# cruiseresearchgroup/ViLCo

Measured on AMD Instinct MI355X. Metric: clips/sec (fwd+bwd) MQ transformer T=2304 C=2304, higher is better.
Workload: dtype fp16 MFMA on 2-part splits of power-of-two scaled fp32 operands (22 significant bits, 3 MFMAs per product), fp32 accumulate: fp32-equivalent; weight-gradient products with contraction length >= 2048 use the leading fp16 parts only (11-bit operands, 1 MFMA; <= 3.5e-4 of the 3-MFMA gradients at this c; 1 GPU; MQ ViLCo backbone config P: T=2304 Cin=2304 D=1024 H=16 arch(2,2,5) XLNet layer text L=77x768 22 classes, train mode with the reference's dropout 0.1 / droppath 0.1 / XLNet dropout 0.1 (mq_vilco.yaml, xlnet_config_1024.json); clips_per_gpu=2, global_batch=2, parallelism=dp1

## Files before the change

### include/vilco_hip.h

```cpp
#ifndef VILCO_HIP_H
#define VILCO_HIP_H

#include <stddef.h>
#include <stdint.h>

#ifdef __cplusplus
extern "C" {
#endif

enum vilco_status {
  VILCO_OK = 0,
  VILCO_ERR_BADARG = -1,
  VILCO_ERR_UNSUPPORTED = -2,
  VILCO_ERR_LAUNCH = -3,
  VILCO_ERR_WORKSPACE = -4
};

const char* vilco_status_str(int status);
const char* vilco_version(void);
size_t vilco_abi_sizeof(const char* struct_name);

enum { VILCO_ACT_NONE = 0, VILCO_ACT_RELU = 1, VILCO_ACT_GELU = 2 };
enum { VILCO_TAP_NONE = 0, VILCO_TAP_A = 1, VILCO_TAP_B = 2 };

// ... 252 lines not shown
                    float* partial, float* norm_coef, void* stream);
typedef struct vilco_optim_desc {
  int32_t kind;
  const int64_t* ptrs;
  const int64_t* numel;
  const int32_t* chunk_tensor;
  const int64_t* chunk_off;
  const int32_t* group;
  int32_t n, nchunks, chunk;
  const float* lr;
  const float* wd;
  int32_t ngroups;
  float beta1, beta2, eps, momentum;
  const float* tensor_step;
  const float* norm_coef;
  float* chunk_amax;
  const float* lr_dev;
} vilco_optim_desc;
int vilco_optim_step(const vilco_optim_desc* d, void* stream);
int vilco_store_f32(float* dst, const float* vals, int32_t n, void* stream);

int vilco_qkv_pre_supported(int32_t C);
int vilco_qkv_pre_amax_parts(int32_t B, int32_t T, int32_t stride);
int vilco_qkv_pre_fwd(const float* x, const float* ln1_g, const float* ln1_b, const float* const* w,
                      const float* const* gam, const float* const* bet, const int32_t* len, float* h,
                      float* const* y, float* mean1, float* rstd1, float* const* mean, float* const* rstd,
                      float* const* amax_parts, int32_t B, int32_t T, int32_t C, int32_t stride, float eps1, float eps,
                      void* stream);
size_t vilco_qkv_pre_bwd_workspace(int32_t B, int32_t T, int32_t C, int32_t stride);
int vilco_qkv_pre_bwd(const float* h, const float* const* w, const float* const* gam, const float* const* dy,
                      const float* const* mean, const float* const* rstd, const int32_t* len,
                      const float* dh_ext, float* const* dc, float* dh, float* dparams, int32_t B, int32_t T,
                      int32_t C, int32_t stride, void* workspace, size_t workspace_bytes, void* stream);

typedef struct vilco_loss_desc {
  const float* logits;
  const float* offsets;
  const float* level_scale;
  const float* points;
  const int32_t* row_level;
  const int32_t* row_pos;
  const int32_t* level_len;
  const float* gt;
  const float* gauss;
  float* loss_norm;
  int32_t B, R, C, L, Nmax;
  float center_radius, label_smoothing, momentum, loss_weight, al_weight;
  int32_t use_al;
} vilco_loss_desc;
size_t vilco_mq_loss_workspace(int32_t B, int32_t R, int32_t C);
int vilco_mq_loss_fwd(const vilco_loss_desc* d, float* out, float* saved, void* almax_state, void* workspace,
                      size_t workspace_bytes, void* stream);
int vilco_mq_loss_bwd(const vilco_loss_desc* d, const float* g_cls, const float* g_reg, const float* g_al,
                      const float* g_final, const float* saved, const void* workspace, float* d_logits,
                      float* d_offsets, float* d_level_scale, float* d_gauss, void* stream);

typedef struct vilco_distill_desc {
  const float* logits;
  const float* targets;
  const int32_t* level_row;
  const int32_t* level_T;
  const int32_t* level_dev;
  int32_t B, R, C, L;
  int32_t clip;
  int32_t ldt;
  int32_t n_known;
// ... 138 lines not shown
```

### vilco_amd/_lib.py

```python
import ctypes as C
import os

_HERE = os.path.dirname(os.path.abspath(__file__))
LIB_PATH = os.environ.get("VILCO_HIP_LIB") or os.path.join(_HERE, "libvilco_hip.so")

ACT_NONE, ACT_RELU, ACT_GELU = 0, 1, 2
TAP_NONE, TAP_A, TAP_B = 0, 1, 2

c_fp = C.c_void_p
i32, i64, f32, sz = C.c_int32, C.c_int64, C.c_float, C.c_size_t


class GemmDesc(C.Structure):
    _cname_ = "vilco_gemm_desc"
    _fields_ = [
        ("A", c_fp), ("B", c_fp), ("C", c_fp),
        ("M", i32), ("N", i32), ("K", i32),
        ("a_kcontig", i32), ("b_kcontig", i32),
        ("lda", i64), ("ldb", i64), ("ldc", i64),
        ("batch_outer", i32), ("batch_inner", i32),
        ("sAo", i64), ("sAi", i64), ("sBo", i64), ("sBi", i64), ("sCo", i64), ("sCi", i64),
        ("tap_operand", i32), ("tapC", i32), ("tapT", i32),
        ("precision", i32),
        ("alpha", f32), ("beta", f32),
# ... 70 lines not shown
                ("rows", i64), ("C", i32), ("drop_p", f32), ("drop_seed", C.c_uint32),
                ("workspace", c_fp), ("workspace_bytes", sz), ("amax_parts", c_fp), ("n_parts", c_fp),
                ("dy_amax", c_fp), ("n_dy_amax", i32), ("planes", c_fp), ("planes_bytes", sz), ("seq_len", i32),
                ("row_mask", c_fp)]


class OptimDesc(C.Structure):
    _cname_ = "vilco_optim_desc"
    _fields_ = [("kind", i32), ("ptrs", c_fp), ("numel", c_fp), ("chunk_tensor", c_fp), ("chunk_off", c_fp), ("group", c_fp),
                ("n", i32), ("nchunks", i32), ("chunk", i32), ("lr", c_fp), ("wd", c_fp), ("ngroups", i32),
                ("beta1", f32), ("beta2", f32), ("eps", f32), ("momentum", f32), ("tensor_step", c_fp), ("norm_coef", c_fp),
                ("chunk_amax", c_fp), ("lr_dev", c_fp)]


class DistillDesc(C.Structure):
    _cname_ = "vilco_distill_desc"
    _fields_ = [("logits", c_fp), ("targets", c_fp), ("level_row", c_fp), ("level_T", c_fp), ("level_dev", c_fp),
                ("B", i32), ("R", i32), ("C", i32), ("L", i32), ("clip", i32), ("ldt", i32), ("n_known", i32), ("mode", i32),
                ("scale", f32)]


class BicCorrectDesc(C.Structure):
    _cname_ = "vilco_bic_correct_desc"
    _fields_ = [("x", c_fp), ("y", c_fp), ("splits", c_fp), ("table", c_fp), ("rows", i64), ("C", i32), ("S", i32),
                ("ldx", i32), ("ldy", i32), ("n_layers", i32)]


class PromptDesc(C.Structure):
    _cname_ = "vilco_prompt_desc"
    _fields_ = [("x", c_fp), ("prompt", c_fp), ("key", c_fp), ("cls", c_fp), ("idx_in", c_fp),
                ("B", i32), ("L", i32), ("C", i32), ("P", i32), ("len", i32), ("k", i32), ("key_mode", i32), ("vote", i32),
                ("idx", c_fp), ("sim", c_fp), ("pn", c_fp), ("xn", c_fp), ("selkey", c_fp), ("prompted", c_fp),
                ("reduce_sim", c_fp), ("workspace", c_fp), ("workspace_bytes", sz)]


SIGNATURES = {
    "vilco_status_str": (C.c_char_p, [C.c_int]),
    "vilco_version": (C.c_char_p, []),
    "vilco_abi_sizeof": (sz, [C.c_char_p]),
    "vilco_defer_set": (C.c_int, [i32]),
    "vilco_defer_pending": (i64, []),
    "vilco_defer_flush": (C.c_int, [c_fp]),
    "vilco_gemm_workspace": (sz, [C.POINTER(GemmDesc)]),
    "vilco_gemm": (C.c_int, [C.POINTER(GemmDesc), c_fp]),
    "vilco_gemm_group": (C.c_int, [C.POINTER(GemmDesc), i32, c_fp]),
    "vilco_gemm_amax_parts": (i32, [C.POINTER(GemmDesc)]),
    "vilco_gemm_force": (C.c_int, [i32, i32]),
    "vilco_gemm_set_skinny": (C.c_int, [i32]),
    "vilco_gemm_config_gen": (i64, []),
    "vilco_gemm_profile_begin": (C.c_int, []),
    "vilco_gemm_profile_end": (C.c_int, [C.POINTER(C.c_double), C.POINTER(C.c_int64)]),
    "vilco_gemm_profile_records": (C.c_int64, [C.POINTER(C.c_int64), C.POINTER(C.c_double), C.c_int64]),
    "vilco_pack_bytes": (sz, [i64, i64, i32]),
    "vilco_pack_item_bytes": (sz, [C.POINTER(PackItem), i32]),
    "vilco_pack": (C.c_int, [c_fp, i64, i64, i64, i32, c_fp, sz, c_fp]),
    "vilco_pack_many": (C.c_int, [C.POINTER(PackItem), i32, i32, c_fp]),
    "vilco_layernorm_fwd": (C.c_int, [C.POINTER(LnFwdDesc), c_fp]),
    "vilco_layernorm_planes_bytes": (sz, [i64, i32, i32]),
    "vilco_layernorm_bwd_workspace": (sz, [i64, i32]),
    "vilco_layernorm_bwd": (C.c_int, [C.POINTER(LnBwdDesc), c_fp]),
    "vilco_dwconv3_fwd": (C.c_int, [c_fp, c_fp, c_fp, c_fp, i32, i32, i32, i32, c_fp]),
    "vilco_dwconv3_bwd_workspace": (sz, [i32, i32, i32, i32]),
    "vilco_dwconv3_bwd": (C.c_int, [c_fp, c_fp, c_fp, c_fp, c_fp, c_fp, i32, i32, i32, i32, c_fp, sz, c_fp]),
    "vilco_maxpool3s2_fwd": (C.c_int, [c_fp, c_fp, c_fp, i32, i32, i32, c_fp]),
    "vilco_maxpool3s2_bwd": (C.c_int, [c_fp, c_fp, c_fp, c_fp, i32, i32, i32, c_fp]),
    "vilco_softmax_fwd": (C.c_int, [c_fp, c_fp, i32, i32, i32, i32, i32, c_fp]),
# ... 10 lines not shown
    "vilco_attn_dsplanes_bytes": (sz, [i32, i32, i32]),
    "vilco_xl_scores_workspace": (sz, [i32, i32, i32, i32]),
    "vilco_xl_scores": (C.c_int, [c_fp, c_fp, c_fp, i32, i32, i32, i32, i32, i32, c_fp, sz, c_fp]),
    "vilco_decode_workspace": (sz, [i32, i32]),
    "vilco_decode": (C.c_int, [c_fp, c_fp, c_fp, c_fp, c_fp, i32, i32, i32, f32, f32, c_fp, c_fp, c_fp, c_fp, c_fp, sz, c_fp]),
    "vilco_scale_add_fwd": (C.c_int, [c_fp, c_fp, c_fp, c_fp, c_fp, c_fp, i32, i32, i32, i32, c_fp]),
    "vilco_colsum_workspace": (sz, [i64, i32]),
    "vilco_scale_add_bwd": (C.c_int, [C.POINTER(ScaleAddBwdDesc), c_fp]),
    "vilco_dropout": (C.c_int, [c_fp, c_fp, i64, f32, C.c_uint32, C.c_uint64, c_fp]),
    "vilco_attn_dropout_mask": (C.c_int, [c_fp, i64, i32, f32, C.c_uint32, c_fp]),
    "vilco_seed_word_set": (C.c_int, [C.c_uint32, c_fp]),
    "vilco_seed_word_bump": (C.c_int, [c_fp]),
    "vilco_seed_word_get": (C.c_int, [C.POINTER(C.c_uint32)]),
    "vilco_axpby": (C.c_int, [c_fp, c_fp, c_fp, f32, f32, i64, c_fp]),
    "vilco_act_bwd": (C.c_int, [C.POINTER(ActBwdDesc), c_fp]),
    "vilco_act_bwd_planes_bytes": (sz, [i64, i32, i32]),
    "vilco_colsum": (C.c_int, [c_fp, c_fp, i64, i32, c_fp, sz, c_fp]),
    "vilco_mask_rows": (C.c_int, [c_fp, c_fp, i32, i32, i32, c_fp]),
    "vilco_add_pe": (C.c_int, [c_fp, c_fp, c_fp, c_fp, i32, i32, i32, c_fp]),
    "vilco_transpose2d": (C.c_int, [c_fp, c_fp, i32, i32, i32, c_fp]),
    "vilco_permute3": (C.c_int, [c_fp, c_fp, i32, i32, i32, i64, i64, i64, i64, c_fp]),
    "vilco_grad_norm": (C.c_int, [c_fp, c_fp, c_fp, c_fp, i32, i32, i32, f32, c_fp, c_fp, c_fp]),
    "vilco_optim_step": (C.c_int, [C.POINTER(OptimDesc), c_fp]),
    "vilco_store_f32": (C.c_int, [c_fp, C.POINTER(f32), i32, c_fp]),
    "vilco_qkv_pre_supported": (C.c_int, [i32]),
    "vilco_qkv_pre_amax_parts": (C.c_int, [i32, i32, i32]),
    "vilco_qkv_pre_fwd": (C.c_int, [c_fp, c_fp, c_fp, C.POINTER(c_fp), C.POINTER(c_fp), C.POINTER(c_fp), c_fp, c_fp,
                                    C.POINTER(c_fp), c_fp, c_fp, C.POINTER(c_fp), C.POINTER(c_fp), C.POINTER(c_fp), i32, i32,
                                    i32, i32, f32, f32, c_fp]),
    "vilco_qkv_pre_bwd_workspace": (sz, [i32, i32, i32, i32]),
    "vilco_qkv_pre_bwd": (C.c_int, [c_fp, C.POINTER(c_fp), C.POINTER(c_fp), C.POINTER(c_fp), C.POINTER(c_fp),
                                    C.POINTER(c_fp), c_fp, c_fp, C.POINTER(c_fp), c_fp, c_fp, i32, i32, i32, i32, c_fp, sz,
                                    c_fp]),
    "vilco_mq_loss_workspace": (sz, [i32, i32, i32]),
    "vilco_mq_loss_fwd": (C.c_int, [C.POINTER(LossDesc), c_fp, c_fp, c_fp, c_fp, sz, c_fp]),
    "vilco_mq_loss_bwd": (C.c_int, [C.POINTER(LossDesc), c_fp, c_fp, c_fp, c_fp, c_fp, c_fp, c_fp, c_fp, c_fp, c_fp,
                                    c_fp]),
    "vilco_cl_distill_workspace": (sz, [i64]),
    "vilco_cl_distill_fwd": (C.c_int, [C.POINTER(DistillDesc), c_fp, c_fp, sz, c_fp]),
    "vilco_cl_distill_bwd": (C.c_int, [C.POINTER(DistillDesc), c_fp, c_fp, c_fp]),
    "vilco_cl_penalty": (C.c_int, [c_fp, c_fp, c_fp, c_fp, i32, i32, i32, f32, i32, c_fp, c_fp, c_fp]),
    "vilco_cl_accumulate": (C.c_int, [c_fp, c_fp, c_fp, c_fp, i32, i32, i32, i32, f32, f32, c_fp]),
    "vilco_nms_workspace": (sz, [i64, i32]),
    "vilco_nms_1d": (C.c_int, [c_fp, c_fp, c_fp, i32, i64, f32, c_fp, c_fp, c_fp, sz, c_fp]),
    "vilco_softnms_1d": (C.c_int, [c_fp, c_fp, c_fp, i32, i64, f32, f32, f32, i32, i64, c_fp, c_fp, c_fp,
                                   c_fp, sz, c_fp]),
    "vilco_nms_set_kernel": (C.c_int, [i32]),
    "vilco_nms_last_kernels": (C.c_int, []),
    "vilco_det_ap_workspace": (sz, [i64, i32, i32]),
    "vilco_det_ap": (C.c_int, [c_fp, c_fp, c_fp, c_fp, c_fp, i64, c_fp, c_fp, c_fp, c_fp, c_fp, i32, i32, c_fp, i32, i32,
                               C.POINTER(C.c_double), i32, c_fp, c_fp, c_fp, sz, c_fp]),
    "vilco_retrieval_hits_workspace": (sz, [i32, i32, i32]),
    "vilco_retrieval_hits": (C.c_int, [c_fp, c_fp, c_fp, c_fp, c_fp, c_fp, c_fp, i32, C.POINTER(C.c_double), i32,
                                       C.POINTER(i32), i32, c_fp, c_fp, c_fp, sz, c_fp]),
    "vilco_score_fuse_workspace": (sz, [i64, i32]),
    "vilco_score_fuse": (C.c_int, [c_fp, c_fp, c_fp, C.POINTER(i32), i64, i32, c_fp, i32, i32, i32, C.POINTER(i32), i64,
                                   c_fp, c_fp, c_fp, c_fp, c_fp, c_fp, sz, c_fp]),
    "vilco_nlq_recall_workspace": (sz, [i64, i32]),
    "vilco_nlq_recall": (C.c_int, [c_fp, i32, c_fp, i32, c_fp, c_fp, i64, i32, C.POINTER(C.c_double), i32, C.POINTER(i32), i32,
                                   i32, c_fp, c_fp, c_fp, c_fp, c_fp, c_fp, sz, c_fp]),
    "vilco_nlq_ensemble": (C.c_int, [c_fp, i32, c_fp, i32, i64, i32, i32, i32, C.c_double, C.c_double, i32, i32, c_fp, c_fp,
                                     c_fp, c_fp, c_fp]),
    "vilco_frob_scale_workspace": (sz, [i64, i64]),
    "vilco_frob_scale": (C.c_int, [c_fp, i64, i64, i64, c_fp, c_fp, sz, c_fp]),
    "vilco_gram_workspace": (sz, [i64, i64]),
    "vilco_gram": (C.c_int, [c_fp, i64, i64, i64, c_fp, c_fp, i32, c_fp, sz, c_fp]),
# ... 51 lines not shown
```

### vilco_amd/csrc/qkvpre.hip

```cpp
#include <cstdlib>
#include "common.h"

void vilco_reduce_rows(const float* ws, float* out0, float* out1, int nrows, int ncols, int split, hipStream_t s);

namespace {

constexpr int QT = 256;

struct QkvArgs {
  const float* x;
  const float* g1; const float* b1;
  const float* w[3];
  const float* gam[3]; const float* bet[3];
  const int* len;
  float* h;
  float* y[3];
  float* mean1; float* rstd1;
  float* mean[3]; float* rstd[3];
  float* amax[3];
  int B, T, Tout, C, stride, seg;
  float eps1, eps;
};

template <int N, int NW>
// ... 609 lines not shown
#pragma unroll
  for (int i = 0; i < 6; ++i) p[(long)i * C + c] = acc[i];
#pragma unroll
  for (int j = 0; j < 3; ++j)
#pragma unroll
    for (int k = 0; k < 3; ++k) p[(long)(6 + 3 * j) * C + c * 3 + k] = acc[6 + 3 * j + k];
}

__global__ __launch_bounds__(QT) void qkv_pre_bwd_dh_kernel(QkvBwdArgs a, const float* __restrict__ dh_ext, float* __restrict__ dh) {
  const int C = a.C, C4 = C >> 2, s = a.stride;
  const long total = (long)a.B * a.T * C4;
  for (long i = (long)blockIdx.x * blockDim.x + threadIdx.x; i < total; i += (long)gridDim.x * blockDim.x) {
    const int c = (int)(i % C4) * 4;
    const long bt = i / C4;
    const int t = (int)(bt % a.T), b = (int)(bt / a.T);
    float4 o = dh_ext ? *reinterpret_cast<const float4*>(dh_ext + bt * C + c) : make_float4(0.f, 0.f, 0.f, 0.f);
#pragma unroll
    for (int tap = 0; tap < 3; ++tap) {
      const int num = t + 1 - tap;
      if (num < 0 || (num % s) != 0) continue;
      const int to = num / s;
      if (to >= a.Tout) continue;
      const long r = (long)b * a.Tout + to;
#pragma unroll
      for (int j = 0; j < 3; ++j) {
        const float4 g = *reinterpret_cast<const float4*>(a.dc[j] + r * C + c);
        const float* wj = a.w[j] + c * 3 + tap;
        o.x += wj[0] * g.x; o.y += wj[3] * g.y; o.z += wj[6] * g.z; o.w += wj[9] * g.w;
      }
    }
    *reinterpret_cast<float4*>(dh + bt * C + c) = o;
  }
}

int pick_seg(int B, int Tout) {
  int seg = 32;
  while (seg > 4 && (long)B * ((Tout + seg - 1) / seg) < 512) seg >>= 1;
  return seg;
}

bool bad_common(int B, int T, int C, int stride) {
  return B < 0 || T < 0 || C <= 0 || (stride != 1 && stride != 2) || (T % stride) != 0;
}

int param_blocks(long rows) {
  long b = (rows + 31) / 32;
  if (b > 96) b = 96;
  return b < 1 ? 1 : (int)b;
}

}

extern "C" int vilco_qkv_pre_supported(int32_t C) { return C > 0 && (C % 256) == 0 && C / 256 <= 9; }

#define QKV_CASE(KERNEL, CPT_, NT_, GRID, ...) hipLaunchKernelGGL((KERNEL<CPT_, NT_>), GRID, dim3(NT_), 0, s, __VA_ARGS__)
#define QKV_DISPATCH(C_, KERNEL, GRID, ...)                                                                          \
  do {                                                                                                              \
    const int cpt256 = (C_) / 256;                                                                                  \
    if (cpt256 > 4 && (C_) % 768 == 0 && (C_) / 768 <= 4) {                                                         \
      switch ((C_) / 768) {                                                                                         \
        case 1: QKV_CASE(KERNEL, 1, 768, GRID, __VA_ARGS__); break;                                                 \
        case 2: QKV_CASE(KERNEL, 2, 768, GRID, __VA_ARGS__); break;                                                 \
        case 3: QKV_CASE(KERNEL, 3, 768, GRID, __VA_ARGS__); break;                                                 \
        default: QKV_CASE(KERNEL, 4, 768, GRID, __VA_ARGS__); break;                                                \
      }                                                                                                             \
    } else {                                                                                                        \
// ... 106 lines not shown
  return (size_t)param_blocks((long)B * (T / stride)) * 15 * (size_t)C * sizeof(float);
}

extern "C" int vilco_qkv_pre_bwd(const float* h, const float* const* w, const float* const* gam, const float* const* dy,
                                 const float* const* mean, const float* const* rstd, const int32_t* len,
                                 const float* dh_ext, float* const* dc, float* dh, float* dparams, int32_t B, int32_t T,
                                 int32_t C, int32_t stride, void* workspace, size_t workspace_bytes, void* stream) {
  if (!h || !w || !gam || !dy || !mean || !rstd || !len || !dc || !dh || !dparams || bad_common(B, T, C, stride))
    return VILCO_ERR_BADARG;
  if (!vilco_qkv_pre_supported(C)) return VILCO_ERR_UNSUPPORTED;
  if (B == 0 || T == 0) return VILCO_OK;
  if (!workspace || workspace_bytes < vilco_qkv_pre_bwd_workspace(B, T, C, stride)) return VILCO_ERR_WORKSPACE;
  hipStream_t s = reinterpret_cast<hipStream_t>(stream);
  QkvBwdArgs a;
  a.h = h; a.len = len;
  for (int j = 0; j < 3; ++j) {
    if (!w[j] || !dy[j] || !mean[j] || !rstd[j] || !dc[j]) return VILCO_ERR_BADARG;
    a.w[j] = w[j]; a.gam[j] = gam[j]; a.dy[j] = dy[j]; a.mean[j] = mean[j]; a.rstd[j] = rstd[j]; a.dc[j] = dc[j];
  }
  a.B = B; a.T = T; a.Tout = T / stride; a.C = C; a.stride = stride; a.seg = pick_seg(B, a.Tout);
  const dim3 grid((a.Tout + a.seg - 1) / a.seg, B);
  QKV_DISPATCH(C, qkv_pre_bwd_rows_kernel, grid, a);
  const long rows = (long)B * a.Tout;
  const int nb = param_blocks(rows);
  const int rpb = (int)((rows + nb - 1) / nb);
  float* partial = reinterpret_cast<float*>(workspace);
  hipLaunchKernelGGL(qkv_pre_bwd_params_kernel, dim3(nb, (C + QT - 1) / QT), dim3(QT), 0, s, a, partial, rpb);
  vilco_reduce_rows(partial, dparams, nullptr, nb, 15 * C, 15 * C, s);
  long blocks = ((long)B * T * (C / 4) + QT - 1) / QT;
  if (blocks > 4096) blocks = 4096;
  hipLaunchKernelGGL(qkv_pre_bwd_dh_kernel, dim3((int)blocks), dim3(QT), 0, s, a, dh_ext, dh);
  return vilco_launch_status();
}
```

### vilco_amd/csrc/status.hip

```cpp
#include <string.h>
#include "common.h"

extern "C" const char* vilco_status_str(int status) {
  switch (status) {
    case VILCO_OK: return "ok";
    case VILCO_ERR_BADARG: return "vilco_hip: bad argument (null pointer, negative size or misaligned operand)";
    case VILCO_ERR_UNSUPPORTED: return "vilco_hip: shape not supported by the gfx950 kernels";
    case VILCO_ERR_LAUNCH: return "vilco_hip: kernel launch failed";
    case VILCO_ERR_WORKSPACE: return "vilco_hip: workspace too small";
    default: return "vilco_hip: unknown status";
  }
}

extern "C" const char* vilco_version(void) { return "vilco_hip 0.1 gfx950"; }

extern "C" size_t vilco_abi_sizeof(const char* struct_name) {
#define ABI_SIZE(T) if (struct_name && !strcmp(struct_name, #T)) return sizeof(T);
  ABI_SIZE(vilco_gemm_desc) ABI_SIZE(vilco_pack_item) ABI_SIZE(vilco_attn_amax_in) ABI_SIZE(vilco_loss_desc)
  ABI_SIZE(vilco_ln_fwd_desc) ABI_SIZE(vilco_ln_bwd_desc) ABI_SIZE(vilco_attn_desc) ABI_SIZE(vilco_scale_add_bwd_desc)
  ABI_SIZE(vilco_act_bwd_desc) ABI_SIZE(vilco_optim_desc) ABI_SIZE(vilco_distill_desc) ABI_SIZE(vilco_bic_correct_desc)
  ABI_SIZE(vilco_prompt_desc)
#undef ABI_SIZE
  return 0;
}

__device__ int32_t vilco_status_word_storage[16];

int32_t* vilco_status_word_dev() {
  static int32_t* p = [] {
    void* q = nullptr;
    if (hipGetSymbolAddress(&q, HIP_SYMBOL(vilco_status_word_storage)) != hipSuccess) q = nullptr;
    return reinterpret_cast<int32_t*>(q);
  }();
  return p;
}

extern "C" int vilco_status_word_take(int32_t* out) {
  if (!out) return VILCO_ERR_BADARG;
  if (hipDeviceSynchronize() != hipSuccess) return VILCO_ERR_LAUNCH;
  if (hipMemcpyFromSymbol(out, HIP_SYMBOL(vilco_status_word_storage), sizeof(int32_t)) != hipSuccess) return VILCO_ERR_LAUNCH;
  const int32_t zero = 0;
  return hipMemcpyToSymbol(HIP_SYMBOL(vilco_status_word_storage), &zero, sizeof(int32_t)) == hipSuccess ? VILCO_OK : VILCO_ERR_LAUNCH;
}
```

### vilco_amd/ops.py

```python
import ctypes as C
import math
import os

import torch

from . import _lib
from ._lib import ACT_GELU, ACT_NONE, ACT_RELU, TAP_A, TAP_B, TAP_NONE, GemmDesc

_PRECISIONS = {"split": 0, 0: 0, "bf16": 1, 1: 1, "split3": 2, "fp32": 2, 2: 2, "f16x2": 3, 3: 3}
DEFAULT_PRECISION = _PRECISIONS[os.environ.get("VILCO_PRECISION", "f16x2")]
_precision = DEFAULT_PRECISION


_DW = {"f16x1": 4, "f16x2": None}
dw_precision = _DW[os.environ.get("VILCO_DW_PRECISION", "f16x1")]
DW_FAST_MIN_K = 2048


def _dw_prec(prec, K=0):
    return dw_precision if (dw_precision is not None and prec == 3 and K >= DW_FAST_MIN_K) else prec


def set_precision(p=None):
    global _precision
    _precision = DEFAULT_PRECISION if p is None else _PRECISIONS[p]


def arithmetic_key():
    return (int(_precision), -1 if dw_precision is None else int(dw_precision), int(DW_FAST_MIN_K), bool(producer_planes),
            bool(ln_planes), bool(attn_planes), bool(produce_amax), bool(conv_tap_planes), bool(defer_finish), bool(use_qkv_pre),
            tuple(sorted(_FORKS)), int(_dw_fork_rows),
            bool(fold_skip_grads), bool(xl_ds_planes), bool(xl_scores_kernel), bool(linear_group_enabled), bool(use_flash),
            bool(_reuse_packs), bool(_weight_cache), str(range_check), int(_lib.load().vilco_gemm_config_gen()), bool(pack_group_enabled), bool(conv_dz_planes), bool(ln_bwd_amax),
            bool(fused_prompt))


def get_precision():
    return _precision


_raw_stream = getattr(torch._C, "_cuda_getCurrentRawStream", None)


def _stream():
    if _raw_stream is not None:
        return _raw_stream(torch.cuda.current_device())
    return torch.cuda.current_stream().cuda_stream


def _p(t):
    return None if t is None else t.data_ptr()


grad_slot_provider = None


def _grad_out(w):
    if grad_slot_provider is not None:
        slot = grad_slot_provider(w)
        if slot is not None and slot.shape == w.shape and slot.is_contiguous():
            return slot
    return torch.empty_like(w)

# ... 2018 lines not shown
    _chk(ab)
    lib = _lib.load()
    out = torch.empty(3, dtype=torch.float64, device=logits.device)
    nws = lib.vilco_bic_eval_ws_bytes(N, n_clips, int(lo), int(hi))
    ws = _ws(nws, logits.device)
    _lib.check(lib.vilco_bic_eval(logits.data_ptr(), label_bits.data_ptr(), weight.data_ptr(), pos.data_ptr(), clip_ptr.data_ptr(),
                                  N, n_clips, Cn, int(lo), int(hi), float(smoothing), ab.data_ptr(), out.data_ptr(), ws.data_ptr(),
                                  nws, _stream()))
    return out


def bic_fit(logits, label_bits, weight, pos, clip_ptr, order, batch_clips, lo, hi, smoothing, lr, ab):
    N, Cn, n_clips = _bic_cache_args(logits, label_bits, weight, pos, clip_ptr)
    _chk(ab)
    if not order.is_cuda or order.dtype != torch.int32 or not order.is_contiguous():
        raise RuntimeError("order must be a contiguous int32 tensor on the device")
    lib = _lib.load()
    batch_clips = int(batch_clips)
    n_steps = int(order.numel()) // batch_clips if batch_clips > 0 else 0
    losses = torch.empty(n_steps, dtype=torch.float64, device=logits.device)
    nws = lib.vilco_bic_fit_ws_bytes(N, n_clips, batch_clips, int(lo), int(hi))
    ws = _ws(nws, logits.device)
    _lib.check(lib.vilco_bic_fit(logits.data_ptr(), label_bits.data_ptr(), weight.data_ptr(), pos.data_ptr(), clip_ptr.data_ptr(),
                                 N, n_clips, order.data_ptr(), n_steps, batch_clips, Cn, int(lo), int(hi), float(smoothing),
                                 float(lr), ab.data_ptr(), losses.data_ptr(), ws.data_ptr(), nws, _stream()))
    return losses


def qkv_pre_supported(Cn):
    return bool(_lib.load().vilco_qkv_pre_supported(int(Cn)))


use_qkv_pre = os.environ.get("VILCO_QKV_PRE", "1") != "0"


def _ptr3(ts):
    return (_lib.c_fp * 3)(*[_p(t) for t in ts])


class _QkvPre(torch.autograd.Function):

    @staticmethod
    def forward(ctx, x, g1, b1, wq, wk, wv, gq, bq, gk, bk, gv, bv, lens, stride, eps1, eps, want_h, skip=False):
        _chk(x, g1, b1, wq, wk, wv, gq, bq, gk, bk, gv, bv)
        ctx.skip = bool(skip)
        ctx.set_materialize_grads(False)
        lib = _lib.load()
        B, T, Cn = x.shape
        To = T // stride
        dev = x.device
        ys = [torch.empty(B, To, Cn, dtype=torch.float32, device=dev) for _ in range(3)]
        h = torch.empty_like(x) if want_h else None
        stats1 = torch.empty(2, B * T, dtype=torch.float32, device=dev)
        stats = torch.empty(6, B * To, dtype=torch.float32, device=dev)
        means, rstds = [stats[2 * j] for j in range(3)], [stats[2 * j + 1] for j in range(3)]
        npart = lib.vilco_qkv_pre_amax_parts(B, T, int(stride)) if (produce_amax and _precision == 3) else 0
        parts = torch.empty(3, npart, dtype=torch.float32, device=dev) if npart > 0 else None
        _lib.check(lib.vilco_qkv_pre_fwd(x.data_ptr(), _p(g1), _p(b1), _ptr3([wq, wk, wv]), _ptr3([gq, gk, gv]),
                                         _ptr3([bq, bk, bv]), lens.data_ptr(), _p(h), _ptr3(ys), stats1[0].data_ptr(),
                                         stats1[1].data_ptr(), _ptr3(means), _ptr3(rstds),
                                         _ptr3([parts[0], parts[1], parts[2]]) if parts is not None else None, B, T, Cn,
                                         int(stride), float(eps1), float(eps), _stream()))
        if parts is not None:
            for j in range(3):
                _leave(_QkvPre, j, amax=(parts[j], npart))
        ctx.stride, ctx.eps1, ctx.want_h = int(stride), float(eps1), bool(want_h)
        ctx.save_for_backward(x, g1, b1, wq, wk, wv, gq, gk, gv, lens, stats1, stats, h)
        outs = (ys[0], ys[1], ys[2], h) if want_h else (ys[0], ys[1], ys[2])
        return outs + (x,) if skip else outs

    @staticmethod
    def backward(ctx, dq, dk, dv, *more):
        x, g1, b1, wq, wk, wv, gq, gk, gv, lens, stats1, stats, h = ctx.saved_tensors
        more = list(more)
        dh_ext = more.pop(0) if ctx.want_h and more else None
        dskip = more.pop(0) if ctx.skip and more else None
        dskip = None if dskip is None else dskip.contiguous()
        lib = _lib.load()
        B, T, Cn = x.shape
        To = T // ctx.stride
        dev = x.device
        if h is None:
            h = torch.empty_like(x)
            d = _lib.LnFwdDesc(x=x.data_ptr(), gamma=_p(g1), beta=_p(b1), y=h.data_ptr(), rows=B * T, C=Cn, eps=ctx.eps1)
            _lib.check(lib.vilco_layernorm_fwd(C.byref(d), _stream()))
        dys = [torch.zeros(B, To, Cn, dtype=torch.float32, device=dev) if g is None else g.contiguous() for g in (dq, dk, dv)]
        dcs = [torch.empty(B, To, Cn, dtype=torch.float32, device=dev) for _ in range(3)]
        dh = torch.empty_like(x)
        dpar = torch.empty(15, Cn, dtype=torch.float32, device=dev)
        nws = lib.vilco_qkv_pre_bwd_workspace(B, T, Cn, ctx.stride)
        means, rstds = [stats[2 * j] for j in range(3)], [stats[2 * j + 1] for j in range(3)]
        dh_ext = None if dh_ext is None else dh_ext.contiguous()
        dx = torch.empty_like(x)
        dg1 = torch.empty(Cn, dtype=torch.float32, device=dev)
        db1 = torch.empty(Cn, dtype=torch.float32, device=dev)
        with _Deferring(g1, wq, wk, wv, gq, gk, gv) as dfr:
            ws = _ws(nws, dev)
            _lib.check(lib.vilco_qkv_pre_bwd(h.data_ptr(), _ptr3([wq, wk, wv]), _ptr3([gq, gk, gv]), _ptr3(dys), _ptr3(means),
                                             _ptr3(rstds), lens.data_ptr(), _p(dh_ext), _ptr3(dcs), dh.data_ptr(), dpar.data_ptr(),
                                             B, T, Cn, ctx.stride, ws.data_ptr(), nws, _stream()))
            del dcs
            ws1 = _ws(lib.vilco_layernorm_bwd_workspace(B * T, Cn), dev)
            d = _lib.LnBwdDesc(dy=dh.data_ptr(), x=x.data_ptr(), gamma=_p(g1), mean=stats1[0].data_ptr(), rstd=stats1[1].data_ptr(),
                               dres=_p(dskip), dx=dx.data_ptr(), dgamma=dg1.data_ptr(), dbeta=db1.data_ptr(), rows=B * T, C=Cn,
                               workspace=ws1.data_ptr(), workspace_bytes=ws1.numel())
            _lib.check(lib.vilco_layernorm_bwd(C.byref(d), _stream()))
            dfr.hold(dpar, dg1, db1)
        dws = [dpar[6 + 3 * j:9 + 3 * j].view_as(w) for j, w in enumerate((wq, wk, wv))]
        dgs = [dpar[2 * j].view_as(g) for j, g in enumerate((gq, gk, gv))]
        dbs = [dpar[2 * j + 1].view_as(g) for j, g in enumerate((gq, gk, gv))]
        return (dx, dg1.view_as(g1), db1.view_as(g1), dws[0], dws[1], dws[2], dgs[0], dbs[0], dgs[1], dbs[1], dgs[2], dbs[2],
                None, None, None, None, None, None)


# ... 119 lines not shown
```

Baseline: 99.96 clips/s.

## Fuse QKV pre-norm backward with LN1 backward into one streaming kernel

Adds a fused backward kernel for the LN1 -> depthwise conv (q/k/v) -> LN path at stride 2. It recomputes the normalized input on the fly from x and the saved stats, streams over time with a sliding window, and computes the conv/LN gradients, the LN1 input gradient (including skip and external dh), and per-block parameter partials in one pass. This removes the materialized h recompute, the dc/dh intermediates, and the separate LN backward launch, cutting HBM traffic and launch count. In exchange it adds register pressure and serial per-row block reductions, and applies only to stride 2.

Result: no change. 100.8 clips/s (median of 3 runs) (+0.8%).

```diff
diff --git a/include/vilco_hip.h b/include/vilco_hip.h
--- a/include/vilco_hip.h
+++ b/include/vilco_hip.h
@@ -308,6 +308,32 @@
                       const float* const* mean, const float* const* rstd, const int32_t* len,
                       const float* dh_ext, float* const* dc, float* dh, float* dparams, int32_t B, int32_t T,
                       int32_t C, int32_t stride, void* workspace, size_t workspace_bytes, void* stream);
+
+typedef struct vilco_qkv_pre_bwd_desc {
+  const float* x;
+  const float* gamma1;
+  const float* beta1;
+  const float* mean1;
+  const float* rstd1;
+  const float* w[3];
+  const float* gam[3];
+  const float* dy[3];
+  const float* mean[3];
+  const float* rstd[3];
+  const int32_t* len;
+  const float* dh_ext;
+  const float* dskip;
+  float* dx;
+  float* dparams;
+  float* dgamma1;
+  float* dbeta1;
+  int32_t B, T, C, stride;
+  void* workspace;
+  size_t workspace_bytes;
+} vilco_qkv_pre_bwd_desc;
+int vilco_qkv_pre_bwd_fused_supported(int32_t C, int32_t stride);
+size_t vilco_qkv_pre_bwd_fused_workspace(int32_t B, int32_t T, int32_t C, int32_t stride);
+int vilco_qkv_pre_bwd_fused(const vilco_qkv_pre_bwd_desc* d, void* stream);
 
 typedef struct vilco_loss_desc {
   const float* logits;
diff --git a/vilco_amd/_lib.py b/vilco_amd/_lib.py
--- a/vilco_amd/_lib.py
+++ b/vilco_amd/_lib.py
@@ -126,6 +126,15 @@
                 ("B", i32), ("L", i32), ("C", i32), ("P", i32), ("len", i32), ("k", i32), ("key_mode", i32), ("vote", i32),
                 ("idx", c_fp), ("sim", c_fp), ("pn", c_fp), ("xn", c_fp), ("selkey", c_fp), ("prompted", c_fp),
                 ("reduce_sim", c_fp), ("workspace", c_fp), ("workspace_bytes", sz)]
+
+
+class QkvPreBwdDesc(C.Structure):
+    _cname_ = "vilco_qkv_pre_bwd_desc"
+    _fields_ = [("x", c_fp), ("gamma1", c_fp), ("beta1", c_fp), ("mean1", c_fp), ("rstd1", c_fp),
+                ("w", c_fp * 3), ("gam", c_fp * 3), ("dy", c_fp * 3), ("mean", c_fp * 3), ("rstd", c_fp * 3),
+                ("len", c_fp), ("dh_ext", c_fp), ("dskip", c_fp), ("dx", c_fp), ("dparams", c_fp), ("dgamma1", c_fp),
+                ("dbeta1", c_fp), ("B", i32), ("T", i32), ("C", i32), ("stride", i32),
+                ("workspace", c_fp), ("workspace_bytes", sz)]
 
 
 SIGNATURES = {
@@ -202,6 +211,9 @@
     "vilco_qkv_pre_bwd": (C.c_int, [c_fp, C.POINTER(c_fp), C.POINTER(c_fp), C.POINTER(c_fp), C.POINTER(c_fp),
                                     C.POINTER(c_fp), c_fp, c_fp, C.POINTER(c_fp), c_fp, c_fp, i32, i32, i32, i32, c_fp, sz,
                                     c_fp]),
+    "vilco_qkv_pre_bwd_fused_supported": (C.c_int, [i32, i32]),
+    "vilco_qkv_pre_bwd_fused_workspace": (sz, [i32, i32, i32, i32]),
+    "vilco_qkv_pre_bwd_fused": (C.c_int, [C.POINTER(QkvPreBwdDesc), c_fp]),
     "vilco_mq_loss_workspace": (sz, [i32, i32, i32]),
     "vilco_mq_loss_fwd": (C.c_int, [C.POINTER(LossDesc), c_fp, c_fp, c_fp, c_fp, sz, c_fp]),
     "vilco_mq_loss_bwd": (C.c_int, [C.POINTER(LossDesc), c_fp, c_fp, c_fp, c_fp, c_fp, c_fp, c_fp, c_fp, c_fp, c_fp,
diff --git a/vilco_amd/csrc/qkvpre.hip b/vilco_amd/csrc/qkvpre.hip
--- a/vilco_amd/csrc/qkvpre.hip
+++ b/vilco_amd/csrc/qkvpre.hip
@@ -665,6 +665,292 @@
     *reinterpret_cast<float4*>(dh + bt * C + c) = o;
   }
 }
+
+struct QkvFusedArgs {
+  const float* x; const float* g1; const float* b1; const float* mean1; const float* rstd1;
+  const float* w[3]; const float* gam[3]; const float* dy[3]; const float* mean[3]; const float* rstd[3];
+  const int* len; const float* dh_ext; const float* dskip;
+  float* dx; float* partial;
+  int B, T, Tout, C, seg;
+};
+
+__device__ __forceinline__ void ld4a(const float* p, float (&v)[4]) {
+  const float4 t = ldg4(p);
+  v[0] = t.x; v[1] = t.y; v[2] = t.z; v[3] = t.w;
+}
+__device__ __forceinline__ void st4a(float* p, const float (&v)[4]) { stg4(p, make_float4(v[0], v[1], v[2], v[3])); }
+
+template <int NW, int S>
+__global__ __launch_bounds__(NW * 64) void qkv_pre_bwd_fused_kernel(QkvFusedArgs a) {
+  constexpr int NP = S;
+  constexpr int NS = 6 + 2 * NP;
+  constexpr int DW = 4 - S;
+  __shared__ float red[NW * NS];
+  const int b = blockIdx.y, t0 = blockIdx.x * a.seg;
+  const int t1 = t0 + a.seg < a.Tout ? t0 + a.seg : a.Tout;
+  const int C = a.C, T = a.T, Tout = a.Tout, c0 = threadIdx.x * 4;
+  const float invC = 1.f / (float)C;
+  const int len = a.len[b];
+
+  float w[3][3][4], gam[3][4], g1[4], b1[4];
+#pragma unroll
+  for (int j = 0; j < 3; ++j) {
+    float t[12];
+    const float4 wa = ldg4(a.w[j] + c0 * 3), wb = ldg4(a.w[j] + c0 * 3 + 4), wc = ldg4(a.w[j] + c0 * 3 + 8);
+    t[0] = wa.x; t[1] = wa.y; t[2] = wa.z; t[3] = wa.w; t[4] = wb.x; t[5] = wb.y; t[6] = wb.z; t[7] = wb.w;
+    t[8] = wc.x; t[9] = wc.y; t[10] = wc.z; t[11] = wc.w;
+#pragma unroll
+    for (int k = 0; k < 4; ++k) {
+      w[j][0][k] = t[k * 3]; w[j][1][k] = t[k * 3 + 1]; w[j][2][k] = t[k * 3 + 2];
+      gam[j][k] = 1.f;
+    }
+    if (a.gam[j]) ld4a(a.gam[j] + c0, gam[j]);
+  }
+#pragma unroll
+  for (int k = 0; k < 4; ++k) { g1[k] = 1.f; b1[k] = 0.f; }
+  if (a.g1) ld4a(a.g1 + c0, g1);
+  if (a.b1) ld4a(a.b1 + c0, b1);
+
+  float acc[17][4];
+#pragma unroll
+  for (int i = 0; i < 17; ++i)
+#pragma unroll
+    for (int k = 0; k < 4; ++k) acc[i][k] = 0.f;
+
+  const float* xb = a.x + (long)b * T * C + c0;
+  const float* m1 = a.mean1 + (long)b * T;
+  const float* r1 = a.rstd1 + (long)b * T;
+
+  float xr[S][4], xmu[S], xrs[S], dyr[3][4], dmu[3], drs[3];
+  auto fetch = [&](int u) {
+#pragma unroll
+    for (int r = 0; r < S; ++r) {
+      int row = S == 1 ? u + 1 : 2 * u + r;
+      row = row < 0 ? 0 : (row >= T ? T - 1 : row);
+      ld4a(xb + (long)row * C, xr[r]);
+      xmu[r] = m1[row]; xrs[r] = r1[row];
+    }
+    const int uc = u < 0 ? 0 : (u >= Tout ? Tout - 1 : u);
+    const long ro = (long)b * Tout + uc;
+#pragma unroll
+    for (int j = 0; j < 3; ++j) {
+      ld4a(a.dy[j] + ro * C + c0, dyr[j]);
+      dmu[j] = a.mean[j][ro]; drs[j] = a.rstd[j][ro];
+    }
+  };
+  auto norm_row = [&](int row, const float (&xv)[4], float mu, float rs, float (&xh)[4], float (&h)[4]) {
+    const bool in = row >= 0 && row < T;
+#pragma unroll
+    for (int k = 0; k < 4; ++k) {
+      xh[k] = (xv[k] - mu) * rs;
+      h[k] = in ? xh[k] * g1[k] + b1[k] : 0.f;
+    }
+  };
+
+  float xw[3][4], hw[3][4], rsw[3];
+  float dcw[DW][3][4];
+  float pg[NP][4], pxh[NP][4], prs[NP];
+  int prow[NP]; bool pown[NP];
+#pragma unroll
+  for (int p = 0; p < NP; ++p) {
+    prs[p] = 0.f; prow[p] = 0; pown[p] = false;
+#pragma unroll
+    for (int k = 0; k < 4; ++k) { pg[p][k] = 0.f; pxh[p][k] = 0.f; }
+  }
+#pragma unroll
+  for (int d = 0; d < DW; ++d)
+#pragma unroll
+    for (int j = 0; j < 3; ++j)
+#pragma unroll
+      for (int k = 0; k < 4; ++k) dcw[d][j][k] = 0.f;
+
+  const int u_lo = S == 1 ? t0 - 1 : t0, u_hi = t1;
+  {
+    constexpr int Q0 = S == 1 ? 1 : 2;
+#pragma unroll
+    for (int q = 0; q < 3; ++q) {
+      if (q < Q0) {
+        rsw[q] = 0.f;
+#pragma unroll
+        for (int k = 0; k < 4; ++k) { xw[q][k] = 0.f; hw[q][k] = 0.f; }
+      } else {
+        const int row = S * u_lo - 1 + (q - Q0);
+        const int rc = row < 0 ? 0 : (row >= T ? T - 1 : row);
+        float xv[4];
+        ld4a(xb + (long)rc * C, xv);
+        rsw[q] = r1[rc];
+        norm_row(row, xv, m1[rc], rsw[q], xw[q], hw[q]);
+      }
+    }
+  }
+  fetch(u_lo);
+
+  auto finish = [&](const auto& sm, int off, const float (&sk)[NP][4]) {
+#pragma unroll
+    for (int p = 0; p < NP; ++p)
+      if (pown[p]) {
+        const float s1 = sm[off + 2 * p] * invC, s2 = sm[off + 2 * p + 1] * invC;
+        float o[4];
+#pragma unroll
+        for (int k = 0; k < 4; ++k) o[k] = prs[p] * (pg[p][k] - s1 - pxh[p][k] * s2) + sk[p][k];
+        st4a(a.dx + ((long)b * T + prow[p]) * C + c0, o);
+      }
+  };
+  auto load_skip = [&](float (&sk)[NP][4]) {
+#pragma unroll
+    for (int p = 0; p < NP; ++p) {
+#pragma unroll
+      for (int k = 0; k < 4; ++k) sk[p][k] = 0.f;
+      if (a.dskip && pown[p]) ld4a(a.dskip + ((long)b * T + prow[p]) * C + c0, sk[p]);
+    }
+  };
+
+  for (int u = u_lo; u <= u_hi; ++u) {
+    if (S == 1) {
+      rsw[0] = rsw[1]; rsw[1] = rsw[2];
+#pragma unroll
+      for (int k = 0; k < 4; ++k) { xw[0][k] = xw[1][k]; hw[0][k] = hw[1][k]; xw[1][k] = xw[2][k]; hw[1][k] = hw[2][k]; }
+      rsw[2] = xrs[0];
+      norm_row(u + 1, xr[0], xmu[0], xrs[0], xw[2], hw[2]);
+    } else {
+      rsw[0] = rsw[2];
+#pragma unroll
+      for (int k = 0; k < 4; ++k) { xw[0][k] = xw[2][k]; hw[0][k] = hw[2][k]; }
+      rsw[1] = xrs[0]; rsw[2] = xrs[S - 1];
+      norm_row(2 * u, xr[0], xmu[0], xrs[0], xw[1], hw[1]);
+      norm_row(2 * u + 1, xr[S - 1], xmu[S - 1], xrs[S - 1], xw[2], hw[2]);
+    }
+    float dyv[3][4], mu[3], rs[3];
+#pragma unroll
+    for (int j = 0; j < 3; ++j) {
+      mu[j] = dmu[j]; rs[j] = drs[j];
+#pragma unroll
+      for (int k = 0; k < 4; ++k) dyv[j][k] = dyr[j][k];
+    }
+    float sk[NP][4], ext[NP][4];
+    load_skip(sk);
+    int nrow[NP]; bool nown[NP];
+    if (S == 1) { nrow[0] = u - 1; nown[0] = u - 1 >= t0 && u - 1 < t1; }
+    else { nrow[0] = 2 * u - 1; nown[0] = u > t0; nrow[NP - 1] = 2 * u; nown[NP - 1] = u < t1; }
+#pragma unroll
+    for (int p = 0; p < NP; ++p) {
+#pragma unroll
+      for (int k = 0; k < 4; ++k) ext[p][k] = 0.f;
+      if (a.dh_ext && nown[p]) ld4a(a.dh_ext + ((long)b * T + nrow[p]) * C + c0, ext[p]);
+    }
+    fetch(u + 1);
+
+    const bool inr = u >= 0 && u < Tout, valid = inr && S * u < len;
+    float g[3][4], xh[3][4], sm[NS];
+#pragma unroll
+    for (int i = 0; i < NS; ++i) sm[i] = 0.f;
+#pragma unroll
+    for (int j = 0; j < 3; ++j)
+#pragma unroll
+      for (int k = 0; k < 4; ++k) {
+        const float cv = valid ? w[j][0][k] * hw[0][k] + w[j][1][k] * hw[1][k] + w[j][2][k] * hw[2][k] : 0.f;
+        xh[j][k] = (cv - mu[j]) * rs[j];
+        g[j][k] = dyv[j][k] * gam[j][k];
+        sm[2 * j] += g[j][k];
+        sm[2 * j + 1] += g[j][k] * xh[j][k];
+      }
+#pragma unroll
+    for (int p = 0; p < NP; ++p)
+#pragma unroll
+      for (int k = 0; k < 4; ++k) {
+        sm[6 + 2 * p] += pg[p][k];
+        sm[6 + 2 * p + 1] += pg[p][k] * pxh[p][k];
+      }
+    block_sums<NS, NW>(sm, red);
+    finish(sm, 6, sk);
+
+#pragma unroll
+    for (int d = 0; d + 1 < DW; ++d)
+#pragma unroll
+      for (int j = 0; j < 3; ++j)
+#pragma unroll
+        for (int k = 0; k < 4; ++k) dcw[d][j][k] = dcw[d + 1][j][k];
+    const bool own = u >= t0 && u < t1;
+#pragma unroll
+    for (int j = 0; j < 3; ++j) {
+      const float s1 = sm[2 * j] * invC, s2 = sm[2 * j + 1] * invC;
+#pragma unroll
+      for (int k = 0; k < 4; ++k) {
+        const float dc = valid ? rs[j] * (g[j][k] - s1 - xh[j][k] * s2) : 0.f;
+        dcw[DW - 1][j][k] = dc;
+        if (own) {
+          acc[2 * j][k] += dyv[j][k] * xh[j][k];
+          acc[2 * j + 1][k] += dyv[j][k];
+          acc[6 + 3 * j][k] += dc * hw[0][k];
+          acc[6 + 3 * j + 1][k] += dc * hw[1][k];
+          acc[6 + 3 * j + 2][k] += dc * hw[2][k];
+        }
+      }
+    }
+
+#pragma unroll
+    for (int p = 0; p < NP; ++p) {
+      pown[p] = nown[p]; prow[p] = nrow[p];
+      const int q = (S == 1) ? 0 : p;
+      prs[p] = rsw[q];
+#pragma unroll
+      for (int k = 0; k < 4; ++k) {
+        float dh = ext[p][k];
+        if (S == 1) {
+#pragma unroll
+          for (int j = 0; j < 3; ++j) dh += w[j][0][k] * dcw[2][j][k] + w[j][1][k] * dcw[1][j][k] + w[j][2][k] * dcw[0][j][k];
+        } else if (p == 0) {
+#pragma unroll
+          for (int j = 0; j < 3; ++j) dh += w[j][2][k] * dcw[0][j][k] + w[j][0][k] * dcw[DW - 1][j][k];
+        } else {
+#pragma unroll
+          for (int j = 0; j < 3; ++j) dh += w[j][1][k] * dcw[DW - 1][j][k];
+        }
+        if (!nown[p]) dh = 0.f;
+        pxh[p][k] = xw[q][k];
+        pg[p][k] = dh * g1[k];
+        acc[15][k] += dh * xw[q][k];
+        acc[16][k] += dh;
+      }
+    }
+  }
+  {
+    float sk[NP][4], sm[2 * NP];
+    load_skip(sk);
+#pragma unroll
+    for (int p = 0; p < NP; ++p) {
+      sm[2 * p] = 0.f; sm[2 * p + 1] = 0.f;
+#pragma unroll
+      for (int k = 0; k < 4; ++k) { sm[2 * p] += pg[p][k]; sm[2 * p + 1] += pg[p][k] * pxh[p][k]; }
+    }
+    block_sums<2 * NP, NW>(sm, red);
+    finish(sm, 0, sk);
+  }
+
+  float* pp = a.partial + ((long)blockIdx.y * gridDim.x + blockIdx.x) * 17 * C;
+#pragma unroll
+  for (int i = 0; i < 6; ++i) st4a(pp + (long)i * C + c0, acc[i]);
+#pragma unroll
+  for (int j = 0; j < 3; ++j) {
+    float t[12];
+#pragma unroll
+    for (int k = 0; k < 4; ++k) { t[k * 3] = acc[6 + 3 * j][k]; t[k * 3 + 1] = acc[6 + 3 * j + 1][k]; t[k * 3 + 2] = acc[6 + 3 * j + 2][k]; }
+    float* q = pp + (long)(6 + 3 * j) * C + c0 * 3;
+    stg4(q, make_float4(t[0], t[1], t[2], t[3]));
+    stg4(q + 4, make_float4(t[4], t[5], t[6], t[7]));
+    stg4(q + 8, make_float4(t[8], t[9], t[10], t[11]));
+  }
+  st4a(pp + (long)15 * C + c0, acc[15]);
+  st4a(pp + (long)16 * C + c0, acc[16]);
+}
+
+int fused_seg(int B, int Tout) {
+  int per_clip = 256 / (B > 0 ? B : 1);
+  if (per_clip < 1) per_clip = 1;
+  const int seg = (Tout + per_clip - 1) / per_clip;
+  return seg < 8 ? 8 : seg;
+}
+int fused_blocks(int B, int Tout) { const int seg = fused_seg(B, Tout); return (Tout + seg - 1) / seg; }
 
 int pick_seg(int B, int Tout) {
   int seg = 32;
@@ -837,3 +1123,47 @@
   hipLaunchKernelGGL(qkv_pre_bwd_dh_kernel, dim3((int)blocks), dim3(QT), 0, s, a, dh_ext, dh);
   return vilco_launch_status();
 }
+
+extern "C" int vilco_qkv_pre_bwd_fused_supported(int32_t C, int32_t stride) {
+  return C > 0 && (C % 256) == 0 && C / 256 <= 4 && (stride == 1 || stride == 2);
+}
+
+extern "C" size_t vilco_qkv_pre_bwd_fused_workspace(int32_t B, int32_t T, int32_t C, int32_t stride) {
+  if (bad_common(B, T, C, stride) || B == 0 || T == 0) return 0;
+  return (size_t)B * fused_blocks(B, T / stride) * 17 * (size_t)C * sizeof(float);
+}
+
+extern "C" int vilco_qkv_pre_bwd_fused(const vilco_qkv_pre_bwd_desc* d, void* stream) {
+  if (!d) return VILCO_ERR_BADARG;
+  const int32_t B = d->B, T = d->T, C = d->C, stride = d->stride;
+  if (!d->x || !d->mean1 || !d->rstd1 || !d->len || !d->dx || !d->dparams || !d->dgamma1 || !d->dbeta1 ||
+      bad_common(B, T, C, stride))
+    return VILCO_ERR_BADARG;
+  for (int j = 0; j < 3; ++j)
+    if (!d->w[j] || !d->dy[j] || !d->mean[j] || !d->rstd[j]) return VILCO_ERR_BADARG;
+  if (d->dbeta1 != d->dgamma1 + C) return VILCO_ERR_BADARG;
+  if (!vilco_qkv_pre_bwd_fused_supported(C, stride)) return VILCO_ERR_UNSUPPORTED;
+  if (B == 0 || T == 0) return VILCO_OK;
+  bool al = vilco_aligned(d->x, 16) && vilco_aligned(d->gamma1, 16) && vilco_aligned(d->beta1, 16) && vilco_aligned(d->dx, 16) &&
+            vilco_aligned(d->dh_ext, 16) && vilco_aligned(d->dskip, 16) && vilco_aligned(d->workspace, 16);
+  for (int j = 0; j < 3; ++j) al = al && vilco_aligned(d->w[j], 16) && vilco_aligned(d->gam[j], 16) && vilco_aligned(d->dy[j], 16);
+  if (!al) return VILCO_ERR_BADARG;
+  if (!d->workspace || d->workspace_bytes < vilco_qkv_pre_bwd_fused_workspace(B, T, C, stride)) return VILCO_ERR_WORKSPACE;
+  hipStream_t s = reinterpret_cast<hipStream_t>(stream);
+  QkvFusedArgs a;
+  a.x = d->x; a.g1 = d->gamma1; a.b1 = d->beta1; a.mean1 = d->mean1; a.rstd1 = d->rstd1;
+  for (int j = 0; j < 3; ++j) {
+    a.w[j] = d->w[j]; a.gam[j] = d->gam[j]; a.dy[j] = d->dy[j]; a.mean[j] = d->mean[j]; a.rstd[j] = d->rstd[j];
+  }
+  a.len = d->len; a.dh_ext = d->dh_ext; a.dskip = d->dskip; a.dx = d->dx;
+  a.partial = reinterpret_cast<float*>(d->workspace);
+  a.B = B; a.T = T; a.Tout = T / stride; a.C = C; a.seg = fused_seg(B, a.Tout);
+  const dim3 grid(fused_blocks(B, a.Tout), B);
+#define FUSED_CASE(N) \
+  case N: if (stride == 1) hipLaunchKernelGGL((qkv_pre_bwd_fused_kernel<N, 1>), grid, dim3(N * 64), 0, s, a); \
+          else hipLaunchKernelGGL((qkv_pre_bwd_fused_kernel<N, 2>), grid, dim3(N * 64), 0, s, a); break
+  switch (C / 256) { FUSED_CASE(1); FUSED_CASE(2); FUSED_CASE(3); default: FUSED_CASE(4); }
+#undef FUSED_CASE
+  vilco_reduce_rows(a.partial, d->dparams, d->dgamma1, (int)(grid.x * grid.y), 17 * C, 15 * C, s);
+  return vilco_launch_status();
+}
diff --git a/vilco_amd/csrc/status.hip b/vilco_amd/csrc/status.hip
--- a/vilco_amd/csrc/status.hip
+++ b/vilco_amd/csrc/status.hip
@@ -19,7 +19,7 @@
   ABI_SIZE(vilco_gemm_desc) ABI_SIZE(vilco_pack_item) ABI_SIZE(vilco_attn_amax_in) ABI_SIZE(vilco_loss_desc)
   ABI_SIZE(vilco_ln_fwd_desc) ABI_SIZE(vilco_ln_bwd_desc) ABI_SIZE(vilco_attn_desc) ABI_SIZE(vilco_scale_add_bwd_desc)
   ABI_SIZE(vilco_act_bwd_desc) ABI_SIZE(vilco_optim_desc) ABI_SIZE(vilco_distill_desc) ABI_SIZE(vilco_bic_correct_desc)
-  ABI_SIZE(vilco_prompt_desc)
+  ABI_SIZE(vilco_prompt_desc) ABI_SIZE(vilco_qkv_pre_bwd_desc)
 #undef ABI_SIZE
   return 0;
 }
diff --git a/vilco_amd/ops.py b/vilco_amd/ops.py
--- a/vilco_amd/ops.py
+++ b/vilco_amd/ops.py
@@ -28,7 +28,7 @@
 
 def arithmetic_key():
     return (int(_precision), -1 if dw_precision is None else int(dw_precision), int(DW_FAST_MIN_K), bool(producer_planes),
-            bool(ln_planes), bool(attn_planes), bool(produce_amax), bool(conv_tap_planes), bool(defer_finish), bool(use_qkv_pre),
+            bool(ln_planes), bool(attn_planes), bool(produce_amax), bool(conv_tap_planes), bool(defer_finish), bool(use_qkv_pre), bool(qkv_bwd_fused), tuple(qkv_bwd_fused_strides),
             tuple(sorted(_FORKS)), int(_dw_fork_rows),
             bool(fold_skip_grads), bool(xl_ds_planes), bool(xl_scores_kernel), bool(linear_group_enabled), bool(use_flash),
             bool(_reuse_packs), bool(_weight_cache), str(range_check), int(_lib.load().vilco_gemm_config_gen()), bool(pack_group_enabled), bool(conv_dz_planes), bool(ln_bwd_amax),
@@ -2113,6 +2113,12 @@
 
 
 use_qkv_pre = os.environ.get("VILCO_QKV_PRE", "1") != "0"
+qkv_bwd_fused = True
+qkv_bwd_fused_strides = (2,)
+
+
+def qkv_pre_bwd_fused_supported(Cn, stride):
+    return bool(_lib.load().vilco_qkv_pre_bwd_fused_supported(int(Cn), int(stride)))
 
 
 def _ptr3(ts):
@@ -2161,6 +2167,27 @@
         B, T, Cn = x.shape
         To = T // ctx.stride
         dev = x.device
+        if qkv_bwd_fused and ctx.stride in qkv_bwd_fused_strides and qkv_pre_bwd_fused_supported(Cn, ctx.stride):
+            dys = [torch.zeros(B, To, Cn, dtype=torch.float32, device=dev) if g is None else g.contiguous() for g in (dq, dk, dv)]
+            dh_ext = None if dh_ext is None else dh_ext.contiguous()
+            dpar = torch.empty(17, Cn, dtype=torch.float32, device=dev)
+            dx = torch.empty_like(x)
+            nws = lib.vilco_qkv_pre_bwd_fused_workspace(B, T, Cn, ctx.stride)
+            with _Deferring(g1, wq, wk, wv, gq, gk, gv) as dfr:
+                ws = _ws(nws, dev)
+                d = _lib.QkvPreBwdDesc(x=x.data_ptr(), gamma1=_p(g1), beta1=_p(b1), mean1=stats1[0].data_ptr(),
+                                       rstd1=stats1[1].data_ptr(), w=_ptr3([wq, wk, wv]), gam=_ptr3([gq, gk, gv]), dy=_ptr3(dys),
+                                       mean=_ptr3([stats[0], stats[2], stats[4]]), rstd=_ptr3([stats[1], stats[3], stats[5]]),
+                                       len=lens.data_ptr(), dh_ext=_p(dh_ext), dskip=_p(dskip), dx=dx.data_ptr(),
+                                       dparams=dpar.data_ptr(), dgamma1=dpar[15].data_ptr(), dbeta1=dpar[16].data_ptr(),
+                                       B=B, T=T, C=Cn, stride=ctx.stride, workspace=ws.data_ptr(), workspace_bytes=nws)
+                _lib.check(lib.vilco_qkv_pre_bwd_fused(C.byref(d), _stream()))
+                dfr.hold(dpar)
+            dws = [dpar[6 + 3 * j:9 + 3 * j].view_as(w) for j, w in enumerate((wq, wk, wv))]
+            dgs = [dpar[2 * j].view_as(g) for j, g in enumerate((gq, gk, gv))]
+            dbs = [dpar[2 * j + 1].view_as(g) for j, g in enumerate((gq, gk, gv))]
+            return (dx, dpar[15].view_as(g1), dpar[16].view_as(g1), dws[0], dws[1], dws[2], dgs[0], dbs[0], dgs[1], dbs[1],
+                    dgs[2], dbs[2], None, None, None, None, None, None)
         if h is None:
             h = torch.empty_like(x)
             d = _lib.LnFwdDesc(x=x.data_ptr(), gamma=_p(g1), beta=_p(b1), y=h.data_ptr(), rows=B * T, C=Cn, eps=ctx.eps1)
```
